# microsoft/tutel

Hardware: AMD Instinct MI355X
Metric: MoE-layer fwd tokens/sec, 4096 tok x H=2048 x E=64 top-2 (higher is better)
Workload: dtype bf16

## Files before the change

### tutel_amd/csrc/common.h

```cpp
#pragma once
#include <hip/hip_runtime.h>
#include <stdint.h>
#include <stdio.h>
#include <string.h>

#include "../../include/tutel_amd.h"

#define WAVE 64

void tutel_set_error(const char *fmt, ...);
int tutel_get_option(int key);

int tutel_stage_begin(int stage, hipStream_t st);
void tutel_stage_end(int token, hipStream_t st);
void tutel_stage_hint(int stage);
void tutel_gemm_corun_hint(int on);
int tutel_gemm_corun();
void tutel_stage_range_push(int stage);
void tutel_stage_range_pop();
struct StageScope {
  int token;
  hipStream_t st;
  StageScope(int stage, hipStream_t s) : token(tutel_stage_begin(stage, s)), st(s) { tutel_stage_range_push(stage); }
  ~StageScope() {
    tutel_stage_end(token, st);
    tutel_stage_range_pop();
  }
};

#define EP_NCAN 16
struct PeerCanary {
  const uint32_t *epoch;
  long long off;
  int world;
  int stale;
};
struct EncodePeer {
  const uint64_t *tab;
  long long off;
  int rank, rows;
  int slot0;
  PeerCanary can;
};
int tutel_encode_launch(const void *x, int dtype, const int32_t *slot_map, const void *gates, int gate_dtype, int T, int M,
                        int n_slots, int capacity, int num_experts, int chunk_rows, int expert_slice, int ep_world, void *out,
                        const EncodePeer &peer, hipStream_t st);
struct GemmProblem {
  const void *A = nullptr; int64_t a_stride_e = 0, a_stride_w = 0; int a_rows_per_w = 0, lda = 0;
  const void *W = nullptr; int64_t w_stride_e = 0; int ldw = 0;
  const void *bias = nullptr; int64_t bias_stride_e = 0;
  void *D = nullptr; int64_t d_stride_e = 0, d_stride_w = 0; int d_rows_per_w = 0, ldd = 0;
  int E_loc = 0, R = 0, N = 0, K = 0;
  int dtype = -1;
  const int32_t *row_counts = nullptr; int row_align = 1;
  const int32_t *a_rows = nullptr; int a_rows_mod = 0; const void *a_zero = nullptr;
  const void *mul = nullptr;
  const uint64_t *d_peer = nullptr; int64_t d_peer_off = 0; const PeerCanary *d_can = nullptr;
  const uint8_t *fl_idx8 = nullptr; int fl_n = 0; int32_t *fl_loc = nullptr;
};
static inline void gemm_one_rank(GemmProblem &g, int R) {
  g.R = R;
  g.a_rows_per_w = g.d_rows_per_w = R > 0 ? R : 1;
}
static inline void gemm_gather(GemmProblem &g, const int32_t *slot_map, int T, const void *zero_row) {
  g.a_rows = slot_map; g.a_rows_mod = slot_map != nullptr ? T : 0; g.a_zero = zero_row;
}
int tutel_expert_gemm(const GemmProblem &g, int w_kmajor, int act, hipStream_t st);
int tutel_expert_ffn(const GemmProblem &fc1, const GemmProblem &fc2, int act, int query, hipStream_t st);
struct RouteFinish;
void tutel_route_finish_args(int T, int E, int k, void *ws, RouteFinish *out);
int tutel_decode_finish_launch(const void *buf, int dtype, const int32_t *idx, const int32_t *loc, const void *gates, int gate_dtype, int T, int M,
                               int k, int capacity, int num_experts, void *out, const RouteFinish &fin, hipStream_t st);
#define PK_TILE_ROWS 256
struct PackedTable { const int32_t *off, *tiles, *ntiles, *cap; int tiles_bound; };
int tutel_expert_gemm_packed(const GemmProblem &g, int w_kmajor, int act, const PackedTable &t, const void *w_up, hipStream_t st);
int tutel_decode_packed_launch(const void *buf, int dtype, const int32_t *idx, const int32_t *loc, const void *gates, int gate_dtype, int T,
                               int M, int k, int row_limit, const int32_t *off, void *out, hipStream_t st);
int tutel_gate_topk_launch(const void *in, const float *partials, int splits, int dtype, int T, int E, int k, int normalize_gate,
                           void *logits_out, int32_t *idx, void *gates, void *ws, int32_t *clear_map, int clear_n, uint8_t *idx8,
                           hipStream_t st);
int tutel_route_launch(const tutel_amd_moe_args_t &m, int splits, int32_t *slot_map, tutel_stream_t stream);
static inline bool gate_proj_mixed(int x_dtype, int logits_dtype) {
  return logits_dtype == TUTEL_F32 && (x_dtype == TUTEL_BF16 || x_dtype == TUTEL_F16);
}
int tutel_gate_proj_splits_for(int T, int M, int E, int x_dtype, int logits_dtype);
int tutel_gate_proj_for(const void *x, const void *gate_w, int x_dtype, int logits_dtype, int T, int M, int E, float *partials,
                        size_t partial_bytes, tutel_stream_t stream);

#define TUTEL_REQUIRE(cond, ...)           \
  do {                                     \
    if (!(cond)) {                         \
      tutel_set_error(__VA_ARGS__);        \
      return -1;                           \
    }                                      \
  } while (0)

#define TUTEL_CHECK_LAUNCH(what)                                                    \
  do {                                                                              \
    hipError_t _e = hipGetLastError();                                              \
    if (_e != hipSuccess) {                                                         \
      tutel_set_error("%s: launch failed: %s", what, hipGetErrorString(_e));        \
      return (int)_e;                                                               \
    }                                                                               \
  } while (0)

struct bf16_t { uint16_t v; };
struct f16_t { _Float16 v; };

__device__ __forceinline__ uint16_t f32_to_bf16_bits(float f) {
  uint32_t u = __float_as_uint(f);
  if ((u & 0x7fffffffu) > 0x7f800000u) return 0x7fc0;
  u += 0x7fffu + ((u >> 16) & 1u);
  return (uint16_t)(u >> 16);
}
__device__ __forceinline__ float bf16_bits_to_f32(uint16_t b) {
  return __uint_as_float(((uint32_t)b) << 16);
}

template <typename T> struct Elem;
template <> struct Elem<double> {
  using ct = double;
  static constexpr int dtype = 3;
  __device__ static __forceinline__ double to_f32(double x) { return x; }
  __device__ static __forceinline__ double from_f32(double x) { return x; }
  __device__ static __forceinline__ double eps() { return 2.220446049250313e-16; }
};
template <> struct Elem<float> {
  using ct = float;
  static constexpr int dtype = TUTEL_F32;
  __device__ static __forceinline__ float to_f32(float x) { return x; }
  __device__ static __forceinline__ float from_f32(float x) { return x; }
  __device__ static __forceinline__ float eps() { return 1.1920928955078125e-07f; }
};
template <> struct Elem<bf16_t> {
  using ct = float;
  static constexpr int dtype = TUTEL_BF16;
  __device__ static __forceinline__ float to_f32(bf16_t x) { return bf16_bits_to_f32(x.v); }
  __device__ static __forceinline__ bf16_t from_f32(float x) { return bf16_t{f32_to_bf16_bits(x)}; }
  __device__ static __forceinline__ float eps() { return 0.0078125f; }
};
template <> struct Elem<f16_t> {
  using ct = float;
  static constexpr int dtype = TUTEL_F16;
  __device__ static __forceinline__ float to_f32(f16_t x) { return (float)x.v; }
  __device__ static __forceinline__ f16_t from_f32(float x) { return f16_t{(_Float16)x}; }
  __device__ static __forceinline__ float eps() { return 0.0009765625f; }
};

template <typename T> __device__ __forceinline__ typename Elem<T>::ct round_to(typename Elem<T>::ct x) {
  return Elem<T>::to_f32(Elem<T>::from_f32(x));
}
__device__ __forceinline__ float ct_exp(float x) { return expf(x); }
__device__ __forceinline__ double ct_exp(double x) { return exp(x); }
__device__ __forceinline__ float ct_max(float a, float b) { return fmaxf(a, b); }
__device__ __forceinline__ double ct_max(double a, double b) { return fmax(a, b); }

static inline int dtype_size(int dtype) { return dtype == TUTEL_F32 ? 4 : 2; }
static inline bool dtype_ok(int dtype) {
  return dtype == TUTEL_F32 || dtype == TUTEL_F16 || dtype == TUTEL_BF16;
}

struct __attribute__((aligned(16))) vec16 { uint32_t w[4]; };

template <typename T> struct Vec;
template <> struct Vec<float> {
  static constexpr int N = 4;
  __device__ static __forceinline__ void unpack(const vec16 &v, float *f) {
#pragma unroll
    for (int i = 0; i < 4; ++i) f[i] = __uint_as_float(v.w[i]);
  }
  __device__ static __forceinline__ void pack(const float *f, vec16 &v) {
#pragma unroll
    for (int i = 0; i < 4; ++i) v.w[i] = __float_as_uint(f[i]);
  }
};
template <> struct Vec<bf16_t> {
  static constexpr int N = 8;
  __device__ static __forceinline__ void unpack(const vec16 &v, float *f) {
#pragma unroll
    for (int i = 0; i < 4; ++i) {
      f[2 * i] = __uint_as_float(v.w[i] << 16);
      f[2 * i + 1] = __uint_as_float(v.w[i] & 0xffff0000u);
    }
  }
  __device__ static __forceinline__ void pack(const float *f, vec16 &v) {
#pragma unroll
    for (int i = 0; i < 4; ++i)
      v.w[i] = (uint32_t)f32_to_bf16_bits(f[2 * i]) | ((uint32_t)f32_to_bf16_bits(f[2 * i + 1]) << 16);
  }
};
template <> struct Vec<f16_t> {
  static constexpr int N = 8;
  __device__ static __forceinline__ void unpack(const vec16 &v, float *f) {
#pragma unroll
    for (int i = 0; i < 4; ++i) {
      union { uint32_t u; _Float16 h[2]; } c;
      c.u = v.w[i];
      f[2 * i] = (float)c.h[0];
      f[2 * i + 1] = (float)c.h[1];
    }
  }
  __device__ static __forceinline__ void pack(const float *f, vec16 &v) {
#pragma unroll
    for (int i = 0; i < 4; ++i) {
      union { uint32_t u; _Float16 h[2]; } c;
      c.h[0] = (_Float16)f[2 * i];
      c.h[1] = (_Float16)f[2 * i + 1];
      v.w[i] = c.u;
    }
  }
};

__device__ __forceinline__ float mul_rn(float a, float b) { return __fmul_rn(a, b); }
__device__ __forceinline__ float add_rn(float a, float b) { return __fadd_rn(a, b); }

__device__ __forceinline__ int lane_id() { return (int)(threadIdx.x & 63); }
__device__ __forceinline__ float wave_max(float v) {
#pragma unroll
  for (int o = 32; o > 0; o >>= 1) v = fmaxf(v, __shfl_xor(v, o, 64));
  return v;
}
__device__ __forceinline__ float wave_sum(float v) {
#pragma unroll
  for (int o = 32; o > 0; o >>= 1) v += __shfl_xor(v, o, 64);
  return v;
}

__device__ __forceinline__ void peer_canary_store(const uint64_t *tab, const PeerCanary &c) {
  if (c.epoch == nullptr) return;
  const int nb = (int)gridDim.x, nlast = nb < EP_NCAN ? nb : EP_NCAN, back = nb - 1 - (int)blockIdx.x;
  if (back >= nlast) return;
  __syncthreads();
  const int t = (int)threadIdx.x;
  if (t >= c.world * EP_NCAN) return;
  const int w = t / EP_NCAN, j = t % EP_NCAN;
  if (j % nlast != back) return;
  const uint32_t e = *c.epoch + (c.stale ? 0u : 1u);
  reinterpret_cast<uint32_t *>(tab[w] + c.off)[j] = e;
}
```

### tutel_amd/csrc/routing.hip

```cpp
#include "common.h"
#include "routing_dev.h"
#include "topk_ties.h"

#define GT_THREADS 1024
#define GT_WAVES 16
#define RT_MAX_TILES 128
#define RT_MAX_K 16
#define RT_MAX_E 4096
#define GT_COL_SLAB 1024

static inline int rt_tile(int T) {
  int per = (T + 64 * RT_MAX_TILES - 1) / (64 * RT_MAX_TILES);
  if (per < 1) per = 1;
  return 64 * per;
}
static inline int rt_ntiles(int T) { return (T + rt_tile(T) - 1) / rt_tile(T); }

extern "C" size_t tutel_amd_routing_workspace_bytes(int T, int E, int k) {
  if (T <= 0 || E <= 0 || k <= 0) return 0;
  size_t nt = (size_t)rt_ntiles(T);
  return nt * ((size_t)k * E * sizeof(int32_t) + (size_t)E * sizeof(float));
}

template <typename T, int EPL, int GT_BATCH>
__global__ __launch_bounds__(GT_THREADS) void gate_topk_kernel(
    const T *__restrict__ in, int apply_softmax, int Tn, int E, int k, int normalize, int tile,
    T *__restrict__ scores_out, int32_t *__restrict__ idx, T *__restrict__ gates,
    int32_t *__restrict__ ws_hist, float *__restrict__ ws_colsum, int32_t *__restrict__ clear_map,
    int clear_n, int tie_mode) {
  using CT = typename Elem<T>::ct;
  extern __shared__ __attribute__((aligned(16))) unsigned char smem[];
  int32_t *s_hist = reinterpret_cast<int32_t *>(smem);
  float *s_col = reinterpret_cast<float *>(smem) + (size_t)k * E;
  const int tie_slots = tie_mode > 0 ? tie_mode : GT_WAVES, tie_slot = (int)(threadIdx.x >> 6) % tie_slots;
  CT *s_tv = reinterpret_cast<CT *>(smem + (((size_t)k * E * 4 + 7) & ~(size_t)7)) + (size_t)tie_slot * E;
  uint16_t *s_tp = reinterpret_cast<uint16_t *>(reinterpret_cast<CT *>(smem + (((size_t)k * E * 4 + 7) & ~(size_t)7)) + (size_t)tie_slots * E) +
                   (size_t)tie_slot * E;
  __shared__ int s_lock[GT_WAVES];

  const int tid = threadIdx.x, lane = tid & 63, wid = tid >> 6;
  const int b = blockIdx.x;
  const int t0 = b * tile, t1 = min(Tn, t0 + tile);

  if (clear_map != nullptr) {
    const int per = (clear_n + (int)gridDim.x - 1) / (int)gridDim.x;
    const int c0 = b * per, c1 = min(clear_n, c0 + per);
    for (int i = c0 + tid; i < c1; i += GT_THREADS) clear_map[i] = -1;
  }

  for (int i = tid; i < k * E; i += GT_THREADS) s_hist[i] = 0;
  if (tid < GT_WAVES) s_lock[tid] = 0;
  __syncthreads();

  float colacc[EPL];
#pragma unroll
  for (int j = 0; j < EPL; ++j) colacc[j] = 0.f;

  for (int tb = t0 + wid; tb < t1; tb += GT_WAVES * GT_BATCH) {
    CT v[GT_BATCH][EPL];
    bool live[GT_BATCH];
    int tt[GT_BATCH];
#pragma unroll
    for (int u = 0; u < GT_BATCH; ++u) {
      tt[u] = tb + u * GT_WAVES;
      live[u] = tt[u] < t1;
      const T *row = in + (size_t)min(tt[u], Tn - 1) * E;
#pragma unroll
      for (int j = 0; j < EPL; ++j) {
        int e = lane + 64 * j;
        v[u][j] = (e < E) ? Elem<T>::to_f32(row[e]) : -INFINITY;
      }
    }
    if (apply_softmax) {
      CT m[GT_BATCH], s[GT_BATCH];
#pragma unroll
      for (int u = 0; u < GT_BATCH; ++u) {
        m[u] = -INFINITY;
#pragma unroll
        for (int j = 0; j < EPL; ++j) m[u] = ct_max(m[u], v[u][j]);
      }
#pragma unroll
      for (int o = 32; o > 0; o >>= 1)
#pragma unroll
        for (int u = 0; u < GT_BATCH; ++u) m[u] = ct_max(m[u], __shfl_xor(m[u], o, 64));
#pragma unroll
      for (int u = 0; u < GT_BATCH; ++u) {
        s[u] = 0.f;
#pragma unroll
        for (int j = 0; j < EPL; ++j) {
          int e = lane + 64 * j;
          v[u][j] = (e < E) ? ct_exp(v[u][j] - m[u]) : 0.f;
          s[u] += v[u][j];
        }
      }
#pragma unroll
      for (int o = 32; o > 0; o >>= 1)
#pragma unroll
        for (int u = 0; u < GT_BATCH; ++u) s[u] += __shfl_xor(s[u], o, 64);
#pragma unroll
      for (int u = 0; u < GT_BATCH; ++u)
#pragma unroll
        for (int j = 0; j < EPL; ++j) {
          int e = lane + 64 * j;
          if (e < E) {
            T r = Elem<T>::from_f32(v[u][j] / s[u]);
            v[u][j] = Elem<T>::to_f32(r);
            if (scores_out && live[u]) scores_out[(size_t)tt[u] * E + e] = r;
          } else {
            v[u][j] = -INFINITY;
          }
        }
    }
    unsigned long long nanm[GT_BATCH];
#pragma unroll
    for (int u = 0; u < GT_BATCH; ++u) {
      nanm[u] = 0;
#pragma unroll
      for (int j = 0; j < EPL; ++j) {
        int e = lane + 64 * j;
        if (e < E && live[u]) colacc[j] += (float)v[u][j];
        if (v[u][j] != v[u][j]) { v[u][j] = -INFINITY; nanm[u] |= 1ull << j; }
      }
    }

    unsigned long long taken[GT_BATCH];
    CT myg[GT_BATCH], prev[GT_BATCH];
    int myidx[GT_BATCH];
    bool tied[GT_BATCH];
#pragma unroll
    for (int u = 0; u < GT_BATCH; ++u) { taken[u] = 0; myg[u] = 0; myidx[u] = -1; prev[u] = 0; tied[u] = false; }
    const int rounds = tie_mode ? k + 1 : k;
    for (int c = 0; c < rounds; ++c) {
      CT bv[GT_BATCH];
      int be[GT_BATCH];
#pragma unroll
      for (int u = 0; u < GT_BATCH; ++u) {
        bv[u] = -INFINITY;
        be[u] = 0x7fffffff;
#pragma unroll
        for (int j = 0; j < EPL; ++j) {
          int e = lane + 64 * j;
          bool ok = (e < E) && !((taken[u] >> j) & 1ull);
          if (ok && (v[u][j] > bv[u] || (v[u][j] == bv[u] && e < be[u]))) { bv[u] = v[u][j]; be[u] = e; }
        }
      }
#pragma unroll
      for (int o = 32; o > 0; o >>= 1)
#pragma unroll
        for (int u = 0; u < GT_BATCH; ++u) {
          CT ov = __shfl_xor(bv[u], o, 64);
          int oe = __shfl_xor(be[u], o, 64);
          if (ov > bv[u] || (ov == bv[u] && oe < be[u])) { bv[u] = ov; be[u] = oe; }
        }
#pragma unroll
      for (int u = 0; u < GT_BATCH; ++u) {
        if (c > 0 && bv[u] == prev[u] && be[u] != 0x7fffffff) tied[u] = true;
        prev[u] = bv[u];
        if (c < k) {
          if ((be[u] & 63) == lane) taken[u] |= 1ull << (be[u] >> 6);
          if (lane == c) { myg[u] = bv[u]; myidx[u] = be[u]; }
        }
      }
    }
    if (tie_mode) {
#pragma unroll
      for (int u = 0; u < GT_BATCH; ++u) {
        if (__ballot(nanm[u] != 0ull) != 0ull) tied[u] = true;
        if (tied[u] && live[u]) {
          const bool shared_slot = tie_slots < GT_WAVES;
          if (shared_slot) {
            if (lane == 0)
              while (atomicCAS(&s_lock[tie_slot], 0, 1) != 0) __builtin_amdgcn_s_sleep(2);
            __builtin_amdgcn_fence(__ATOMIC_ACQUIRE, "workgroup");
            __builtin_amdgcn_wave_barrier();
          }
#pragma unroll
          for (int j = 0; j < EPL; ++j) {
            int e = lane + 64 * j;
            if (e < E) {
              s_tv[e] = ((nanm[u] >> j) & 1ull) ? (CT)NAN : v[u][j];
              s_tp[e] = (uint16_t)e;
            }
          }
          __builtin_amdgcn_fence(__ATOMIC_RELEASE, "wavefront");
          __builtin_amdgcn_wave_barrier();
          if constexpr (EPL <= 4) {
            using Rep = typename TkRepOf<T>::type;
            WaveQueue<EPL, Rep> wq;
            wq.sel = reinterpret_cast<uint8_t *>(s_tp);
            wq.seln = E;
#pragma unroll
            for (int j = 0; j < EPL; ++j) wq.r[j] = Rep::make(((nanm[u] >> j) & 1ull) ? (CT)NAN : v[u][j], lane + 64 * j);
            AtenTopk<WaveQueue<EPL, Rep>> tsw(wq);
            tsw.run(E, k);
            if (lane < k) {
              myidx[u] = Rep::id_of(wq.r[0].unpack());
              myg[u] = s_tv[myidx[u]];
            }
          } else {
            if (lane == 0) {
              LdsQueue<CT, uint16_t> lq{s_tv, s_tp};
              AtenTopk<LdsQueue<CT, uint16_t>> ts(lq);
              ts.run(E, k);
            }
            __builtin_amdgcn_fence(__ATOMIC_ACQ_REL, "wavefront");
            __builtin_amdgcn_wave_barrier();
            if (lane < k) {
              myidx[u] = s_tp[lane];
              myg[u] = s_tv[myidx[u]];
            }
          }
          __builtin_amdgcn_fence(__ATOMIC_ACQ_REL, "wavefront");
          __builtin_amdgcn_wave_barrier();
          if (shared_slot) {
            __builtin_amdgcn_fence(__ATOMIC_RELEASE, "workgroup");
            __builtin_amdgcn_wave_barrier();
            if (lane == 0) __hip_atomic_store(&s_lock[tie_slot], 0, __ATOMIC_RELEASE, __HIP_MEMORY_SCOPE_WORKGROUP);
          }
        }
      }
    }
#pragma unroll
    for (int u = 0; u < GT_BATCH; ++u) {
      CT denom = __shfl(myg[u], 0, 64);
      for (int c = 1; c < k; ++c) denom = round_to<T>(denom + __shfl(myg[u], c, 64));
      if (lane < k && live[u]) {
        CT g = myg[u];
        if (normalize && k > 1) {
          CT d = ct_max(denom, (CT)Elem<T>::eps());
          if (denom != denom) d = denom;
          g = g / d;
        }
        gates[(size_t)lane * Tn + tt[u]] = Elem<T>::from_f32(g);
        idx[(size_t)lane * Tn + tt[u]] = myidx[u];
        atomicAdd(&s_hist[lane * E + myidx[u]], 1);
      }
    }
  }

  __syncthreads();
  for (int i = tid; i < k * E; i += GT_THREADS) ws_hist[(size_t)b * k * E + i] = s_hist[i];
  const int slab = E < GT_COL_SLAB ? E : GT_COL_SLAB;
  for (int e0 = 0; e0 < E; e0 += slab) {
#pragma unroll
    for (int j = 0; j < EPL; ++j) {
      int e = lane + 64 * j;
      if (e >= e0 && e < e0 + slab && e < E) s_col[wid * slab + (e - e0)] = colacc[j];
    }
    __syncthreads();
    for (int e = e0 + tid; e < e0 + slab && e < E; e += GT_THREADS) {
      float s = 0.f;
#pragma unroll
      for (int w = 0; w < GT_WAVES; ++w) s += s_col[w * slab + (e - e0)];
      ws_colsum[(size_t)b * E + e] = s;
    }
    __syncthreads();
  }
}

__global__ __launch_bounds__(RT_THREADS) void tile_hist_kernel(const int32_t *__restrict__ idx,
                                                              int Tn, int E, int k, int tile,
                                                              int32_t *__restrict__ ws_hist) {
  extern __shared__ __attribute__((aligned(16))) unsigned char smem[];
  int32_t *s_hist = reinterpret_cast<int32_t *>(smem);
  const int tid = threadIdx.x, b = blockIdx.x;
  const int t0 = b * tile, t1 = min(Tn, t0 + tile);
  for (int i = tid; i < k * E; i += RT_THREADS) s_hist[i] = 0;
  __syncthreads();
  for (int j = 0; j < k; ++j)
    for (int t = t0 + tid; t < t1; t += RT_THREADS) {
      int e = idx[(size_t)j * Tn + t];
      if (e >= 0 && e < E) atomicAdd(&s_hist[j * E + e], 1);
    }
  __syncthreads();
  for (int i = tid; i < k * E; i += RT_THREADS) ws_hist[(size_t)b * k * E + i] = s_hist[i];
}

template <int NW, bool COH = false>
__device__ __forceinline__ void loc_rank(int tid, int t0, int t1, int Tn, int E, int k, const int32_t *__restrict__ idx,
                                         const int32_t *lidx, int lidx_stride, int e_first, bool have_first, int32_t *s_cur,
                                         int32_t *__restrict__ loc, int capacity, int32_t *__restrict__ slot_map) {
  const int lane = tid & 63, wid = tid >> 6;
  int ebits = 0;
  while ((1 << ebits) < E) ++ebits;
  for (int j = wid; j < k; j += NW) {
    int32_t *cur = s_cur + j * E;
    for (int c0 = t0; c0 < t1; c0 += 64) {
      int t = c0 + lane;
      int e;
      if (have_first && j == wid && c0 == t0) e = e_first;
      else if (t >= t1) e = -1;
      else e = lidx != nullptr ? lidx[j * lidx_stride + (t - t0)] : idx[(size_t)j * Tn + t];
      bool valid = (e >= 0) && (e < E);
      unsigned long long same = __ballot(valid);
      for (int bit = 0; bit < ebits; ++bit) {
        const unsigned long long bb = __ballot(valid && ((e >> bit) & 1));
        same &= ((e >> bit) & 1) ? bb : ~bb;
      }
      const int rank = __popcll(same & ((1ull << lane) - 1ull));
      const int cnt = __popcll(same);
      const bool leader = valid && (__ffsll((long long)same) - 1 == lane);
      int base = valid ? cur[e] : 0;
      int l = base + rank;
      if (leader) cur[e] = base + cnt;
      if (t < t1) {
        loc[(size_t)j * Tn + t] = valid ? l : 0;
        if (slot_map != nullptr && valid && l < capacity) st_i32<COH>(slot_map + (size_t)e * capacity + l, j * Tn + t);
      }
    }
  }
}

__global__ __launch_bounds__(RT_THREADS) void location_kernel(
    const int32_t *__restrict__ idx, int Tn, int E, int k, int tile, int ntiles,
    const int32_t *__restrict__ ws_hist, const float *__restrict__ ws_colsum,
    int32_t *__restrict__ loc, int32_t *__restrict__ dispatch_count, int32_t *__restrict__ stats,
    void *__restrict__ l_aux, int l_aux_dtype, int capacity, int32_t *__restrict__ slot_map) {
  extern __shared__ __attribute__((aligned(16))) unsigned char smem[];
  int32_t *s_cur = reinterpret_cast<int32_t *>(smem);
  int32_t *s_tot = s_cur + (size_t)k * E;
  float *s_parts = reinterpret_cast<float *>(smem) + (size_t)2 * k * E;
  __shared__ float s_red[RT_WAVES];
  __shared__ int s_redi[RT_WAVES];

  const int tid = threadIdx.x, lane = tid & 63, wid = tid >> 6;
  const int b = blockIdx.x;
  const int t0 = b * tile, t1 = min(Tn, t0 + tile);

  int e_first = -1;
  if (wid < k && t0 + lane < t1) e_first = idx[(size_t)wid * Tn + t0 + lane];
  const int cs_parts = (E >= RT_THREADS) ? 1 : (RT_THREADS / E);
  const int cs_per = (ntiles + cs_parts - 1) / cs_parts;
  const bool cs_early = b == 0 && l_aux != nullptr && cs_parts * E <= RT_THREADS;
  float cs_first[16];
  if (cs_early && tid < cs_parts * E) {
    const int e = tid % E, a = (tid / E) * cs_per, z = min(ntiles, a + cs_per);
#pragma unroll
    for (int u = 0; u < 16; ++u) cs_first[u] = (a + u < z) ? ws_colsum[(size_t)(a + u) * E + e] : 0.f;
  }
  loc_prefix<RT_WAVES>(tid, b, E, k, ntiles, ws_hist, s_cur, s_tot, dispatch_count);
  loc_rank<RT_WAVES>(tid, t0, t1, Tn, E, k, idx, nullptr, 0, e_first, true, s_cur, loc, capacity, slot_map);
  if (b == 0) loc_finish<RT_WAVES>(tid, Tn, E, k, ntiles, ws_colsum, s_tot, s_parts, s_red, s_redi, cs_first, cs_early, stats, l_aux, l_aux_dtype);
}

#define GQ_LPT 16
#define GQ_THREADS 1024

template <typename V, int N> struct alignas((sizeof(V) * N) > 16 ? 16 : (sizeof(V) * N)) GqPack { V v[N]; };
template <typename V, int N> __device__ __forceinline__ void gq_load(const V *p, V (&o)[N]) {
  const GqPack<V, N> pk = *reinterpret_cast<const GqPack<V, N> *>(p);
#pragma unroll
  for (int i = 0; i < N; ++i) o[i] = pk.v[i];
}

template <typename T, int EPQ>
__global__ __launch_bounds__(GQ_THREADS) void gate_topk_quad_kernel(
    const T *__restrict__ in, int apply_softmax, int Tn, int E, int k, int normalize, int tile,
    T *__restrict__ scores_out, int32_t *__restrict__ idx, T *__restrict__ gates,
    int32_t *__restrict__ ws_hist, float *__restrict__ ws_colsum, int32_t *__restrict__ clear_map,
    int clear_n, const float *__restrict__ part, int nsplit, T *__restrict__ logits_out, uint8_t *__restrict__ idx8, int tie_mode) {
  using CT = typename Elem<T>::ct;
  extern __shared__ __attribute__((aligned(16))) unsigned char smem[];
  const int ES = GQ_LPT * EPQ + 1;
  int32_t *s_hist = reinterpret_cast<int32_t *>(smem);
  float *s_sc = reinterpret_cast<float *>(smem) + (size_t)k * E;
  CT *s_tv = reinterpret_cast<CT *>(smem + ((((size_t)k * E + (size_t)64 * ES) * 4 + 7) & ~(size_t)7));
  uint8_t *s_sel = reinterpret_cast<uint8_t *>(s_tv + (size_t)64 * E) + (size_t)(threadIdx.x >> 6) * 256;
  __shared__ int s_nlist[2];
  __shared__ int s_list[64];

  const int tid = threadIdx.x, q = tid & (GQ_LPT - 1), tl = tid / GQ_LPT;
  const int b = blockIdx.x;
  const int t0 = b * tile, t1 = min(Tn, t0 + tile);

  if (clear_map != nullptr) {
    const int per = (clear_n + (int)gridDim.x - 1) / (int)gridDim.x;
    const int c0 = b * per, c1 = min(clear_n, c0 + per);
    for (int i = c0 + tid; i < c1; i += GQ_THREADS) clear_map[i] = -1;
  }
  for (int i = tid; i < k * E; i += GQ_THREADS) s_hist[i] = 0;
  if (tid < 2) s_nlist[tid] = 0;
  float colsum = 0.f;
  __syncthreads();

  int pass = -1;
  for (int ts = t0; ts < t1; ts += 64) {
    ++pass;
    const int t = ts + tl;
    const bool live = t < t1;
    CT v[EPQ];
    if (part != nullptr) {
      const float *row = part + (size_t)min(t, Tn - 1) * E + q * EPQ;
      const size_t sstride = (size_t)Tn * E;
      const bool exact = E == GQ_LPT * EPQ;
      int ej[EPQ];
#pragma unroll
      for (int j = 0; j < EPQ; ++j) ej[j] = min(q * EPQ + j, E - 1) - q * EPQ;
      float a[EPQ];
#pragma unroll
      for (int j = 0; j < EPQ; ++j) a[j] = 0.f;
#define GQ_PART_SUM(LOAD)                                                                          \
      for (int s0 = 0; s0 < nsplit; s0 += 4) {                                                     \
        float b[4][EPQ];                                                                           \
        _Pragma("unroll") for (int i = 0; i < 4; ++i) {                                            \
          const float *rs = row + (size_t)min(s0 + i, nsplit - 1) * sstride;                       \
          LOAD;                                                                                    \
        }                                                                                          \
        _Pragma("unroll") for (int i = 0; i < 4; ++i)                                              \
          if (s0 + i < nsplit) {                                                                   \
            _Pragma("unroll") for (int j = 0; j < EPQ; ++j) a[j] = (s0 + i == 0) ? b[i][j] : a[j] + b[i][j]; \
          }                                                                                        \
      }
      if (exact) {
        GQ_PART_SUM((gq_load<float, EPQ>(rs, b[i])));
      } else {
        GQ_PART_SUM(_Pragma("unroll") for (int j = 0; j < EPQ; ++j) b[i][j] = rs[ej[j]]);
      }
#undef GQ_PART_SUM
#pragma unroll
      for (int j = 0; j < EPQ; ++j) {
        int e = q * EPQ + j;
        const T r = Elem<T>::from_f32((CT)a[j]);
        if (logits_out && live && e < E) logits_out[(size_t)t * E + e] = r;
        v[j] = (e < E) ? Elem<T>::to_f32(r) : -INFINITY;
      }
    } else {
      const T *row = in + (size_t)min(t, Tn - 1) * E + q * EPQ;
      T raw[EPQ];
      if (E == GQ_LPT * EPQ && (reinterpret_cast<uintptr_t>(in) & 15) == 0) {
        gq_load<T, EPQ>(row, raw);
      } else {
#pragma unroll
        for (int j = 0; j < EPQ; ++j) raw[j] = row[min(q * EPQ + j, E - 1) - q * EPQ];
      }
#pragma unroll
      for (int j = 0; j < EPQ; ++j) {
        int e = q * EPQ + j;
        v[j] = (e < E) ? Elem<T>::to_f32(raw[j]) : -INFINITY;
      }
    }
    if (apply_softmax) {
      CT m = -INFINITY;
#pragma unroll
      for (int j = 0; j < EPQ; ++j) m = ct_max(m, v[j]);
#pragma unroll
      for (int o = 1; o < GQ_LPT; o <<= 1) m = ct_max(m, __shfl_xor(m, o, 64));
      CT s = 0;
#pragma unroll
      for (int j = 0; j < EPQ; ++j) {
        int e = q * EPQ + j;
        v[j] = (e < E) ? ct_exp(v[j] - m) : CT(0);
        s += v[j];
      }
#pragma unroll
      for (int o = 1; o < GQ_LPT; o <<= 1) s += __shfl_xor(s, o, 64);
#pragma unroll
      for (int j = 0; j < EPQ; ++j) {
        int e = q * EPQ + j;
        if (e < E) {
          T r = Elem<T>::from_f32(v[j] / s);
          v[j] = Elem<T>::to_f32(r);
          if (scores_out && live) scores_out[(size_t)t * E + e] = r;
        } else {
          v[j] = -INFINITY;
        }
      }
    }
    uint32_t nanm = 0;
#pragma unroll
    for (int j = 0; j < EPQ; ++j) {
      int e = q * EPQ + j;
      if (e < E) s_sc[tl * ES + e] = live ? (float)v[j] : 0.f;
      if (v[j] != v[j]) { v[j] = -INFINITY; nanm |= 1u << j; }
    }

    uint32_t taken = 0;
    CT myg = 0, prev = 0;
    int myidx = 0;
    bool tied = false;
    const int rounds = tie_mode ? k + 1 : k;
    for (int c = 0; c < rounds; ++c) {
      CT bv = -INFINITY;
      int be = 0x7fffffff;
#pragma unroll
      for (int j = 0; j < EPQ; ++j) {
        int e = q * EPQ + j;
        bool ok = (e < E) && !((taken >> j) & 1u);
        if (ok && (v[j] > bv || (v[j] == bv && e < be))) { bv = v[j]; be = e; }
      }
#pragma unroll
      for (int o = 1; o < GQ_LPT; o <<= 1) {
        CT ov = __shfl_xor(bv, o, 64);
        int oe = __shfl_xor(be, o, 64);
        if (ov > bv || (ov == bv && oe < be)) { bv = ov; be = oe; }
      }
      if (c > 0 && bv == prev && be != 0x7fffffff) tied = true;
      prev = bv;
      if (c < k) {
        if (be / EPQ == q) taken |= 1u << (be - q * EPQ);
        if (c == q) { myg = bv; myidx = be; }
        if (q == 0 && live) {
          idx[(size_t)c * Tn + t] = be;
          if (idx8 != nullptr) idx8[(size_t)c * Tn + t] = (uint8_t)be;
        }
      }
    }
    if (tie_mode) {
      const int rowsh = (int)(threadIdx.x & 48);
      if ((__ballot(nanm != 0) >> rowsh) & 0xffffull) tied = true;
      if (tied && live) {
#pragma unroll
        for (int j = 0; j < EPQ; ++j) {
          int e = q * EPQ + j;
          if (e < E) s_tv[tl * E + e] = ((nanm >> j) & 1u) ? (CT)NAN : v[j];
        }
        if (q == 0) s_list[atomicAdd(&s_nlist[pass & 1], 1)] = tl;
      }
    }
    {
      const int row0 = (int)(threadIdx.x & 48);
      CT denom = __shfl(myg, row0, 64);
      for (int c = 1; c < k; ++c) denom = round_to<T>(denom + __shfl(myg, row0 + c, 64));
      if (q < k && live && !(tie_mode && tied)) {
        CT g = myg;
        if (normalize && k > 1) {
          CT d = ct_max(denom, (CT)Elem<T>::eps());
          if (denom != denom) d = denom;
          g = g / d;
        }
        gates[(size_t)q * Tn + t] = Elem<T>::from_f32(g);
        atomicAdd(&s_hist[q * E + myidx], 1);
      }
    }
    __syncthreads();
    if (tid < E) {
      float s = colsum;
      for (int r = 0; r < 64; ++r) s += s_sc[r * ES + tid];
      colsum = s;
    }
    if (tie_mode) {
      const int wv = (int)(threadIdx.x >> 6), nbusy = (E + 63) >> 6, wl = (int)(threadIdx.x & 63);
      constexpr int SL = (GQ_LPT * EPQ + 63) / 64;
      const int nrep = s_nlist[pass & 1];
      for (int ent = wv - nbusy; ent >= 0 && ent < nrep; ent += GQ_THREADS / 64 - nbusy) {
        const int trow = s_list[ent], tt = ts + trow;
        using Rep = typename TkRepOf<T>::type;
        WaveQueue<SL, Rep> wq;
        wq.sel = s_sel;
        wq.seln = E;
#pragma unroll
        for (int sl = 0; sl < SL; ++sl) {
          const int e = wl + 64 * sl;
          wq.r[sl] = Rep::make(e < E ? s_tv[trow * E + e] : (CT)0, e);
        }
        AtenTopk<WaveQueue<SL, Rep>> tk(wq);
        tk.run(E, k);
        TkElem<CT> res;
        res.id = Rep::id_of(wq.r[0].unpack());
        res.v = s_tv[trow * E + (wl < k ? res.id : 0)];
        CT denom = tk_readlane(res.v, 0);
        for (int c = 1; c < k; ++c) denom = round_to<T>(denom + tk_readlane(res.v, c));
        if (wl < k) {
          CT g = res.v;
          if (normalize && k > 1) {
            CT d = ct_max(denom, (CT)Elem<T>::eps());
            if (denom != denom) d = denom;
            g = g / d;
          }
          gates[(size_t)wl * Tn + tt] = Elem<T>::from_f32(g);
          idx[(size_t)wl * Tn + tt] = res.id;
          if (idx8 != nullptr) idx8[(size_t)wl * Tn + tt] = (uint8_t)res.id;
          atomicAdd(&s_hist[wl * E + res.id], 1);
        }
      }
      if (tid == 0) s_nlist[(pass + 1) & 1] = 0;
    }
    __syncthreads();
  }
  for (int i = tid; i < k * E; i += GQ_THREADS) ws_hist[(size_t)b * k * E + i] = s_hist[i];
  if (tid < E) ws_colsum[(size_t)b * E + tid] = colsum;
}

__global__ __launch_bounds__(256) void slot_map_kernel(const int32_t *__restrict__ idx,
                                                       const int32_t *__restrict__ loc, int n,
                                                       int E, int capacity,
                                                       int32_t *__restrict__ slot_map) {
  int q = blockIdx.x * 256 + threadIdx.x;
  if (q >= n) return;
  int e = idx[q], l = loc[q];
  if (e >= 0 && e < E && l >= 0 && l < capacity) slot_map[(size_t)e * capacity + l] = q;
}

#define CS_WAVES 16
__global__ __launch_bounds__(CS_WAVES * 64) void cumsum_kernel(const int32_t *__restrict__ in,
                                                              int32_t *__restrict__ out, int Tn,
                                                              int E) {
  __shared__ int32_t s_part[CS_WAVES][64];
  const int lane = threadIdx.x & 63, wid = threadIdx.x >> 6;
  const int col = blockIdx.x * 64 + lane;
  const int rows_per = (Tn + CS_WAVES - 1) / CS_WAVES;
  const int r0 = wid * rows_per, r1 = min(Tn, r0 + rows_per);
  int acc = 0;
  if (col < E)
    for (int r = r0; r < r1; ++r) acc += in[(size_t)r * E + col];
  s_part[wid][lane] = acc;
  __syncthreads();
  int run = -1;
  for (int w = 0; w < wid; ++w) run += s_part[w][lane];
  if (col < E)
    for (int r = r0; r < r1; ++r) {
      run += in[(size_t)r * E + col];
      out[(size_t)r * E + col] = run;
    }
}

template <typename T>
static int launch_gate_topk(const void *in, int apply_softmax, int Tn, int E, int k, int normalize,
                            void *scores_out, int32_t *idx, void *gates, void *ws,
                            int32_t *clear_map, int clear_n, hipStream_t st, const float *part = nullptr, int nsplit = 0,
                            void *logits_out = nullptr, uint8_t *idx8 = nullptr) {
  const int tile = rt_tile(Tn), nt = rt_ntiles(Tn);
  int32_t *ws_hist = (int32_t *)ws;
  float *ws_col = (float *)(ws_hist + (size_t)nt * k * E);
  using CTh = typename Elem<T>::ct;
  int tie_mode = tutel_get_option(TUTEL_OPT_TIE_RULE) != 0;
  size_t lds = (size_t)k * E * 4 + 8;
  {
    const size_t col = (size_t)GT_WAVES * (E < GT_COL_SLAB ? E : GT_COL_SLAB) * 4, slot = (size_t)E * (sizeof(CTh) + 2);
    const size_t room = (size_t)160 * 1024 - lds - 256;
    int slots = (int)(room / slot);
    if (slots > GT_WAVES) slots = GT_WAVES;
    if (slots < 1) tie_mode = 0;
    const size_t tie = tie_mode ? (size_t)slots * slot : 0;
    lds += tie > col ? tie : col;
    if (tie_mode && E > 128) tie_mode = slots;
  }
  if (E <= 128) {
    const int epq = (E + GQ_LPT - 1) / GQ_LPT;
    const int epq_t = epq <= 1 ? 1 : (epq <= 2 ? 2 : (epq <= 4 ? 4 : 8));
    const size_t lds_q = ((size_t)k * E + (size_t)64 * (GQ_LPT * epq_t + 1)) * 4 + 8 + (tie_mode ? (size_t)64 * E * sizeof(CTh) + 16 * 256 : 0);
#define GQ_LAUNCH(EPQ)                                                                         \
    do {                                                                                       \
      if (lds_q > 65536) {                                                                     \
        (void)hipFuncSetAttribute((const void *)gate_topk_quad_kernel<T, EPQ>, hipFuncAttributeMaxDynamicSharedMemorySize, (int)lds_q); \
        (void)hipGetLastError();                                                               \
      }                                                                                        \
      hipLaunchKernelGGL((gate_topk_quad_kernel<T, EPQ>), dim3(nt), dim3(GQ_THREADS), lds_q, st,            \
                         (const T *)in, apply_softmax, Tn, E, k, normalize, tile, (T *)scores_out,          \
                         idx, (T *)gates, ws_hist, ws_col, clear_map, clear_n, part, nsplit, (T *)logits_out, idx8, tie_mode); \
    } while (0)
    if (epq_t == 1) GQ_LAUNCH(1);
    else if (epq_t == 2) GQ_LAUNCH(2);
    else if (epq_t == 4) GQ_LAUNCH(4);
    else GQ_LAUNCH(8);
#undef GQ_LAUNCH
    TUTEL_CHECK_LAUNCH("tutel_amd_gate_topk");
    return 0;
  }
  TUTEL_REQUIRE(part == nullptr && idx8 == nullptr, "tutel_amd_gate_topk_partials: E = %d is past the 128 experts the partial-sum form covers", E);
  const int epl = (E + 63) / 64;
#define GT_LAUNCH(EPL)                                                                          \
  do {                                                                                          \
    if (lds > 65536) {                                                                          \
      (void)hipFuncSetAttribute((const void *)gate_topk_kernel<T, EPL, (EPL <= 4 ? 4 : (EPL <= 8 ? 2 : 1))>,                         \
                                hipFuncAttributeMaxDynamicSharedMemorySize, (int)lds);          \
      (void)hipGetLastError();                                                                  \
    }                                                                                           \
    hipLaunchKernelGGL((gate_topk_kernel<T, EPL, (EPL <= 4 ? 4 : (EPL <= 8 ? 2 : 1))>), dim3(nt), dim3(GT_THREADS), lds, st,         \
                       (const T *)in, apply_softmax, Tn, E, k, normalize, tile,                 \
                       (T *)scores_out, idx, (T *)gates, ws_hist, ws_col, clear_map, clear_n, tie_mode);  \
  } while (0)
  if (epl <= 1) GT_LAUNCH(1);
  else if (epl <= 2) GT_LAUNCH(2);
  else if (epl <= 4) GT_LAUNCH(4);
  else if (epl <= 8) GT_LAUNCH(8);
  else if (epl <= 16) GT_LAUNCH(16);
  else if (epl <= 32) GT_LAUNCH(32);
  else GT_LAUNCH(64);
#undef GT_LAUNCH
  TUTEL_CHECK_LAUNCH("tutel_amd_gate_topk");
  return 0;
}

extern "C" int tutel_amd_gate_topk(const void *in, int dtype, int apply_softmax, int T, int E,
                                   int k, int normalize_gate, void *scores_out, int32_t *idx,
                                   void *gates, void *ws, size_t ws_bytes, int32_t *clear_map,
                                   int clear_n, tutel_stream_t stream) {
  TUTEL_REQUIRE(dtype_ok(dtype) || dtype == TUTEL_F64, "tutel_amd_gate_topk: unsupported dtype %d", dtype);
  TUTEL_REQUIRE(T >= 0 && E >= 1 && E <= RT_MAX_E, "tutel_amd_gate_topk: need 1 <= E <= %d (got %d)", RT_MAX_E, E);
  TUTEL_REQUIRE(k >= 1 && k <= RT_MAX_K && k <= E, "tutel_amd_gate_topk: need 1 <= k <= min(E,%d) (got k=%d, E=%d)", RT_MAX_K, k, E);
  TUTEL_REQUIRE((size_t)k * E <= 8192, "tutel_amd_gate_topk: k*E = %d exceeds 8192", k * E);
  if (T == 0) return 0;
  TUTEL_REQUIRE(in && idx && gates && ws, "tutel_amd_gate_topk: null pointer");
  TUTEL_REQUIRE(ws_bytes >= tutel_amd_routing_workspace_bytes(T, E, k), "tutel_amd_gate_topk: workspace too small");
  TUTEL_REQUIRE(clear_n >= 0 && (clear_map != nullptr || clear_n == 0), "tutel_amd_gate_topk: bad clear_map");
  if (clear_n == 0) clear_map = nullptr;
  hipStream_t st = (hipStream_t)stream;
  StageScope stage(TUTEL_STAGE_GATE_TOPK, st);
  if (dtype == TUTEL_F64) return launch_gate_topk<double>(in, apply_softmax, T, E, k, normalize_gate, scores_out, idx, gates, ws, clear_map, clear_n, st);
  if (dtype == TUTEL_F32) return launch_gate_topk<float>(in, apply_softmax, T, E, k, normalize_gate, scores_out, idx, gates, ws, clear_map, clear_n, st);
  if (dtype == TUTEL_BF16) return launch_gate_topk<bf16_t>(in, apply_softmax, T, E, k, normalize_gate, scores_out, idx, gates, ws, clear_map, clear_n, st);
  return launch_gate_topk<f16_t>(in, apply_softmax, T, E, k, normalize_gate, scores_out, idx, gates, ws, clear_map, clear_n, st);
}

void tutel_route_finish_args(int T, int E, int k, void *ws, RouteFinish *out) {
  const int nt = rt_ntiles(T);
  out->Tn = T; out->E = E; out->k = k; out->ntiles = nt;
  out->ws_hist = (const int32_t *)ws;
  out->ws_colsum = (const float *)((const int32_t *)ws + (size_t)nt * k * E);
}

int tutel_gate_topk_launch(const void *in, const float *partials, int splits, int dtype, int T, int E, int k, int normalize_gate,
                           void *logits_out, int32_t *idx, void *gates, void *ws, int32_t *clear_map, int clear_n, uint8_t *idx8,
                           hipStream_t st) {
  TUTEL_REQUIRE(E <= 128 || (partials == nullptr && idx8 == nullptr), "tutel_gate_topk_launch: E = %d is past the 16-lanes-per-token kernel", E);
  if (clear_n == 0) clear_map = nullptr;
  StageScope stage(TUTEL_STAGE_GATE_TOPK, st);
  const int sm = 1;
  if (dtype == TUTEL_F32) return launch_gate_topk<float>(in, sm, T, E, k, normalize_gate, nullptr, idx, gates, ws, clear_map, clear_n, st, partials, splits, logits_out, idx8);
  if (dtype == TUTEL_BF16) return launch_gate_topk<bf16_t>(in, sm, T, E, k, normalize_gate, nullptr, idx, gates, ws, clear_map, clear_n, st, partials, splits, logits_out, idx8);
  return launch_gate_topk<f16_t>(in, sm, T, E, k, normalize_gate, nullptr, idx, gates, ws, clear_map, clear_n, st, partials, splits, logits_out, idx8);
}

extern "C" int tutel_amd_gate_topk_partials(const float *partials, int splits, int dtype, int T, int E, int k,
                                            int normalize_gate, void *logits_out, void *scores_out, int32_t *idx,
                                            void *gates, void *ws, size_t ws_bytes, int32_t *clear_map, int clear_n,
                                            tutel_stream_t stream) {
  TUTEL_REQUIRE(dtype_ok(dtype), "tutel_amd_gate_topk_partials: the logits dtype must be fp32 / fp16 / bf16 (got %d)", dtype);
  TUTEL_REQUIRE(T >= 0 && E >= 1 && E <= 128, "tutel_amd_gate_topk_partials: need 1 <= E <= 128 (got %d)", E);
  TUTEL_REQUIRE(k >= 1 && k <= RT_MAX_K && k <= E, "tutel_amd_gate_topk_partials: need 1 <= k <= min(E,%d) (got k=%d, E=%d)", RT_MAX_K, k, E);
  TUTEL_REQUIRE(splits >= 1 && splits <= 64, "tutel_amd_gate_topk_partials: bad split count %d", splits);
  if (T == 0) return 0;
  TUTEL_REQUIRE(partials && idx && gates && ws, "tutel_amd_gate_topk_partials: null pointer");
  TUTEL_REQUIRE(ws_bytes >= tutel_amd_routing_workspace_bytes(T, E, k), "tutel_amd_gate_topk_partials: workspace too small");
  TUTEL_REQUIRE(clear_n >= 0 && (clear_map != nullptr || clear_n == 0), "tutel_amd_gate_topk_partials: bad clear_map");
  if (clear_n == 0) clear_map = nullptr;
  hipStream_t st = (hipStream_t)stream;
  StageScope stage(TUTEL_STAGE_GATE_TOPK, st);
  if (dtype == TUTEL_F32)
    return launch_gate_topk<float>(nullptr, 1, T, E, k, normalize_gate, scores_out, idx, gates, ws, clear_map, clear_n, st, partials, splits, logits_out);
  if (dtype == TUTEL_BF16)
    return launch_gate_topk<bf16_t>(nullptr, 1, T, E, k, normalize_gate, scores_out, idx, gates, ws, clear_map, clear_n, st, partials, splits, logits_out);
  return launch_gate_topk<f16_t>(nullptr, 1, T, E, k, normalize_gate, scores_out, idx, gates, ws, clear_map, clear_n, st, partials, splits, logits_out);
}

extern "C" int tutel_amd_compute_location(const int32_t *idx, int T, int E, int k, int hist_ready,
                                          void *ws, size_t ws_bytes, int32_t *loc,
                                          int32_t *dispatch_count, int32_t *stats, void *l_aux,
                                          int l_aux_dtype, int capacity, int32_t *slot_map,
                                          int slot_map_cleared, tutel_stream_t stream) {
  TUTEL_REQUIRE(T >= 0 && E >= 1 && E <= RT_MAX_E, "tutel_amd_compute_location: need 1 <= E <= %d (got %d)", RT_MAX_E, E);
  TUTEL_REQUIRE(k >= 1 && k <= RT_MAX_K, "tutel_amd_compute_location: need 1 <= k <= %d (got %d)", RT_MAX_K, k);
  TUTEL_REQUIRE((size_t)k * E <= 8192, "tutel_amd_compute_location: k*E = %d exceeds 8192", k * E);
  TUTEL_REQUIRE(dispatch_count != nullptr, "tutel_amd_compute_location: dispatch_count is null");
  TUTEL_REQUIRE(l_aux == nullptr || dtype_ok(l_aux_dtype), "tutel_amd_compute_location: bad l_aux dtype %d", l_aux_dtype);
  TUTEL_REQUIRE((long long)k * T < 0x7fffffffLL, "tutel_amd_compute_location: k*T overflows int32");
  TUTEL_REQUIRE(hist_ready || l_aux == nullptr, "tutel_amd_compute_location: l_aux needs the column sums written by tutel_amd_gate_topk (hist_ready=1)");
  hipStream_t st = (hipStream_t)stream;
  if (T == 0) {
    (void)hipMemsetAsync(dispatch_count, 0, (size_t)E * 4, st);
    if (stats) (void)hipMemsetAsync(stats, 0, 4, st);
    if (l_aux) (void)hipMemsetAsync(l_aux, 0, dtype_size(l_aux_dtype), st);
    if (slot_map && capacity > 0) (void)hipMemsetAsync(slot_map, 0xFF, (size_t)E * capacity * 4, st);
    return 0;
  }
  TUTEL_REQUIRE(idx && loc && ws, "tutel_amd_compute_location: null pointer");
  TUTEL_REQUIRE(ws_bytes >= tutel_amd_routing_workspace_bytes(T, E, k), "tutel_amd_compute_location: workspace too small");
  const int tile = rt_tile(T), nt = rt_ntiles(T);
  int32_t *ws_hist = (int32_t *)ws;
  float *ws_col = (float *)(ws_hist + (size_t)nt * k * E);
  StageScope stage(TUTEL_STAGE_LOCATION, st);
  if (!hist_ready) {
    hipLaunchKernelGGL(tile_hist_kernel, dim3(nt), dim3(RT_THREADS), (size_t)k * E * 4, st, idx, T, E, k, tile, ws_hist);
    TUTEL_CHECK_LAUNCH("tutel_amd_compute_location(hist)");
  }
  if (slot_map != nullptr && capacity > 0) {
    if (!slot_map_cleared) {
      hipError_t e = hipMemsetAsync(slot_map, 0xFF, (size_t)E * capacity * 4, st);
      TUTEL_REQUIRE(e == hipSuccess, "tutel_amd_compute_location: memset failed: %s", hipGetErrorString(e));
    }
  } else {
    slot_map = nullptr;
    capacity = 0;
  }
  const size_t lds_loc = ((size_t)2 * k * E + (size_t)(E > RT_THREADS ? E : RT_THREADS)) * 4;
  if (lds_loc > 65536) {
    (void)hipFuncSetAttribute((const void *)location_kernel, hipFuncAttributeMaxDynamicSharedMemorySize, (int)lds_loc);
    (void)hipGetLastError();
  }
  hipLaunchKernelGGL(location_kernel, dim3(nt), dim3(RT_THREADS), lds_loc, st, idx, T, E, k,
                     tile, nt, ws_hist, ws_col, loc, dispatch_count, stats, l_aux, l_aux_dtype, capacity, slot_map);
  TUTEL_CHECK_LAUNCH("tutel_amd_compute_location");
  return 0;
}

extern "C" int tutel_amd_slot_map(const int32_t *idx, const int32_t *loc, int T, int E, int k,
                                  int capacity, int32_t *slot_map, tutel_stream_t stream) {
  TUTEL_REQUIRE(E >= 1 && k >= 1 && capacity >= 0 && T >= 0, "tutel_amd_slot_map: bad sizes");
  TUTEL_REQUIRE((long long)k * T < 0x7fffffffLL, "tutel_amd_slot_map: k*T overflows int32");
  hipStream_t st = (hipStream_t)stream;
  if (capacity == 0) return 0;
  TUTEL_REQUIRE(slot_map != nullptr, "tutel_amd_slot_map: null slot_map");
  StageScope stage(TUTEL_STAGE_OTHER, st);
  hipError_t e = hipMemsetAsync(slot_map, 0xFF, (size_t)E * capacity * 4, st);
  TUTEL_REQUIRE(e == hipSuccess, "tutel_amd_slot_map: memset failed: %s", hipGetErrorString(e));
  int n = k * T;
  if (n == 0) return 0;
  TUTEL_REQUIRE(idx && loc, "tutel_amd_slot_map: null pointer");
  hipLaunchKernelGGL(slot_map_kernel, dim3((n + 255) / 256), dim3(256), 0, st, idx, loc, n, E, capacity, slot_map);
  TUTEL_CHECK_LAUNCH("tutel_amd_slot_map");
  return 0;
}

extern "C" int tutel_amd_cumsum_sub_one(const int32_t *mask, int32_t *out, int T, int E,
                                        tutel_stream_t stream) {
  TUTEL_REQUIRE(T >= 0 && E >= 0, "tutel_amd_cumsum_sub_one: bad sizes");
  if (T == 0 || E == 0) return 0;
  TUTEL_REQUIRE(mask && out, "tutel_amd_cumsum_sub_one: null pointer");
  hipLaunchKernelGGL(cumsum_kernel, dim3((E + 63) / 64), dim3(CS_WAVES * 64), 0, (hipStream_t)stream, mask, out, T, E);
  TUTEL_CHECK_LAUNCH("tutel_amd_cumsum_sub_one");
  return 0;
}
```

Before: 16.79 million.

## Prefetch gate rows across passes, use DPP row reductions in top-k kernel

Hoists the per-pass row loads for gate logits and partial sums so that the first pass's loads are issued before the shared-memory clear and each later pass issues its loads at the top of the loop. The 16-lane shuffle reductions for softmax max/sum and the top-k argmax are replaced with DPP row moves (quad xor and row mirrors). The extra tie-detection round is replaced by a ballot check on the remaining candidates. The normalization denominator is now accumulated inside the selection loop rather than gathered by shuffles afterwards. The aim is lower latency in a small routing kernel, at the cost of more live registers and the added complexity of macros and DPP intrinsics.

```diff
diff --git a/tutel_amd/csrc/common.h b/tutel_amd/csrc/common.h
--- a/tutel_amd/csrc/common.h
+++ b/tutel_amd/csrc/common.h
@@ -226,6 +226,23 @@
   return v;
 }
 
+#define DPP_QUAD_XOR1 0xB1
+#define DPP_QUAD_XOR2 0x4E
+#define DPP_ROW_HALF_MIRROR 0x141
+#define DPP_ROW_MIRROR 0x140
+template <int CTRL> __device__ __forceinline__ int dpp_row_move(int x) { return __builtin_amdgcn_update_dpp(0, x, CTRL, 0xf, 0xf, true); }
+template <int CTRL> __device__ __forceinline__ float dpp_row_move(float x) { return __int_as_float(dpp_row_move<CTRL>(__float_as_int(x))); }
+template <int CTRL> __device__ __forceinline__ double dpp_row_move(double x) {
+  return __hiloint2double(dpp_row_move<CTRL>(__double2hiint(x)), dpp_row_move<CTRL>(__double2loint(x)));
+}
+template <typename V, typename Op> __device__ __forceinline__ V row16_all_reduce(V x, Op op) {
+  x = op(x, dpp_row_move<DPP_QUAD_XOR1>(x));
+  x = op(x, dpp_row_move<DPP_QUAD_XOR2>(x));
+  x = op(x, dpp_row_move<DPP_ROW_HALF_MIRROR>(x));
+  x = op(x, dpp_row_move<DPP_ROW_MIRROR>(x));
+  return x;
+}
+
 __device__ __forceinline__ void peer_canary_store(const uint64_t *tab, const PeerCanary &c) {
   if (c.epoch == nullptr) return;
   const int nb = (int)gridDim.x, nlast = nb < EP_NCAN ? nb : EP_NCAN, back = nb - 1 - (int)blockIdx.x;
diff --git a/tutel_amd/csrc/routing.hip b/tutel_amd/csrc/routing.hip
--- a/tutel_amd/csrc/routing.hip
+++ b/tutel_amd/csrc/routing.hip
@@ -353,6 +353,15 @@
   for (int i = 0; i < N; ++i) o[i] = pk.v[i];
 }
 
+template <typename CT> struct GqBest { CT v; int e; };
+template <typename CT> __device__ __forceinline__ GqBest<CT> gq_better(GqBest<CT> a, GqBest<CT> o) {
+  const bool take = (o.v > a.v) | ((o.v == a.v) & (o.e < a.e));
+  return GqBest<CT>{take ? o.v : a.v, take ? o.e : a.e};
+}
+template <int CTRL, typename CT> __device__ __forceinline__ GqBest<CT> dpp_row_move(GqBest<CT> x) {
+  return GqBest<CT>{dpp_row_move<CTRL>(x.v), dpp_row_move<CTRL>(x.e)};
+}
+
 template <typename T, int EPQ>
 __global__ __launch_bounds__(GQ_THREADS) void gate_topk_quad_kernel(
     const T *__restrict__ in, int apply_softmax, int Tn, int E, int k, int normalize, int tile,
@@ -373,6 +382,35 @@
   const int b = blockIdx.x;
   const int t0 = b * tile, t1 = min(Tn, t0 + tile);
 
+  const size_t sstride = (size_t)Tn * E;
+  const bool exact = E == GQ_LPT * EPQ;
+  const bool wide_in = exact && (reinterpret_cast<uintptr_t>(in) & 15) == 0;
+  int ej[EPQ];
+#pragma unroll
+  for (int j = 0; j < EPQ; ++j) ej[j] = min(q * EPQ + j, E - 1) - q * EPQ;
+  float pb[4][EPQ];
+  T raw[EPQ];
+#define GQ_PART_LOAD(S0, LOAD)                                                                     \
+  _Pragma("unroll") for (int i = 0; i < 4; ++i) {                                                  \
+    const float *rs = row + (size_t)min((S0) + i, nsplit - 1) * sstride;                           \
+    LOAD;                                                                                          \
+  }
+#define GQ_LOAD_WIDE gq_load<float, EPQ>(rs, pb[i])
+#define GQ_LOAD_ELEMS _Pragma("unroll") for (int j = 0; j < EPQ; ++j) pb[i][j] = rs[ej[j]]
+#define GQ_PASS_LOADS(TS)                                                                          \
+  do {                                                                                             \
+    const size_t roff = (size_t)min((TS) + tl, Tn - 1) * E + q * EPQ;                              \
+    if (part != nullptr) {                                                                         \
+      const float *row = part + roff;                                                              \
+      if (exact) { GQ_PART_LOAD(0, GQ_LOAD_WIDE) } else { GQ_PART_LOAD(0, GQ_LOAD_ELEMS) }         \
+    } else if (wide_in) {                                                                          \
+      gq_load<T, EPQ>(in + roff, raw);                                                             \
+    } else {                                                                                       \
+      _Pragma("unroll") for (int j = 0; j < EPQ; ++j) raw[j] = in[roff + ej[j]];                   \
+    }                                                                                              \
+  } while (0)
+  GQ_PASS_LOADS(t0);
+
   if (clear_map != nullptr) {
     const int per = (clear_n + (int)gridDim.x - 1) / (int)gridDim.x;
     const int c0 = b * per, c1 = min(clear_n, c0 + per);
@@ -385,38 +423,27 @@
 
   int pass = -1;
   for (int ts = t0; ts < t1; ts += 64) {
-    ++pass;
+    if (++pass > 0) GQ_PASS_LOADS(ts);
     const int t = ts + tl;
     const bool live = t < t1;
     CT v[EPQ];
     if (part != nullptr) {
       const float *row = part + (size_t)min(t, Tn - 1) * E + q * EPQ;
-      const size_t sstride = (size_t)Tn * E;
-      const bool exact = E == GQ_LPT * EPQ;
-      int ej[EPQ];
-#pragma unroll
-      for (int j = 0; j < EPQ; ++j) ej[j] = min(q * EPQ + j, E - 1) - q * EPQ;
       float a[EPQ];
 #pragma unroll
       for (int j = 0; j < EPQ; ++j) a[j] = 0.f;
-#define GQ_PART_SUM(LOAD)                                                                          \
-      for (int s0 = 0; s0 < nsplit; s0 += 4) {                                                     \
-        float b[4][EPQ];                                                                           \
-        _Pragma("unroll") for (int i = 0; i < 4; ++i) {                                            \
-          const float *rs = row + (size_t)min(s0 + i, nsplit - 1) * sstride;                       \
-          LOAD;                                                                                    \
-        }                                                                                          \
-        _Pragma("unroll") for (int i = 0; i < 4; ++i)                                              \
-          if (s0 + i < nsplit) {                                                                   \
-            _Pragma("unroll") for (int j = 0; j < EPQ; ++j) a[j] = (s0 + i == 0) ? b[i][j] : a[j] + b[i][j]; \
-          }                                                                                        \
-      }
+#define GQ_PART_ADD(S0)                                                                           \
+      _Pragma("unroll") for (int i = 0; i < 4; ++i)                                                \
+        if ((S0) + i < nsplit) {                                                                   \
+          _Pragma("unroll") for (int j = 0; j < EPQ; ++j) a[j] = ((S0) + i == 0) ? pb[i][j] : a[j] + pb[i][j]; \
+        }
+      GQ_PART_ADD(0)
       if (exact) {
-        GQ_PART_SUM((gq_load<float, EPQ>(rs, b[i])));
+        for (int s0 = 4; s0 < nsplit; s0 += 4) { GQ_PART_LOAD(s0, GQ_LOAD_WIDE) GQ_PART_ADD(s0) }
       } else {
-        GQ_PART_SUM(_Pragma("unroll") for (int j = 0; j < EPQ; ++j) b[i][j] = rs[ej[j]]);
-      }
-#undef GQ_PART_SUM
+        for (int s0 = 4; s0 < nsplit; s0 += 4) { GQ_PART_LOAD(s0, GQ_LOAD_ELEMS) GQ_PART_ADD(s0) }
+      }
+#undef GQ_PART_ADD
 #pragma unroll
       for (int j = 0; j < EPQ; ++j) {
         int e = q * EPQ + j;
@@ -425,14 +452,6 @@
         v[j] = (e < E) ? Elem<T>::to_f32(r) : -INFINITY;
       }
     } else {
-      const T *row = in + (size_t)min(t, Tn - 1) * E + q * EPQ;
-      T raw[EPQ];
-      if (E == GQ_LPT * EPQ && (reinterpret_cast<uintptr_t>(in) & 15) == 0) {
-        gq_load<T, EPQ>(row, raw);
-      } else {
-#pragma unroll
-        for (int j = 0; j < EPQ; ++j) raw[j] = row[min(q * EPQ + j, E - 1) - q * EPQ];
-      }
 #pragma unroll
       for (int j = 0; j < EPQ; ++j) {
         int e = q * EPQ + j;
@@ -443,8 +462,7 @@
       CT m = -INFINITY;
 #pragma unroll
       for (int j = 0; j < EPQ; ++j) m = ct_max(m, v[j]);
-#pragma unroll
-      for (int o = 1; o < GQ_LPT; o <<= 1) m = ct_max(m, __shfl_xor(m, o, 64));
+      m = row16_all_reduce(m, [](CT x, CT y) { return ct_max(x, y); });
       CT s = 0;
 #pragma unroll
       for (int j = 0; j < EPQ; ++j) {
@@ -452,8 +470,7 @@
         v[j] = (e < E) ? ct_exp(v[j] - m) : CT(0);
         s += v[j];
       }
-#pragma unroll
-      for (int o = 1; o < GQ_LPT; o <<= 1) s += __shfl_xor(s, o, 64);
+      s = row16_all_reduce(s, [](CT x, CT y) { return x + y; });
 #pragma unroll
       for (int j = 0; j < EPQ; ++j) {
         int e = q * EPQ + j;
@@ -475,39 +492,36 @@
     }
 
     uint32_t taken = 0;
-    CT myg = 0, prev = 0;
+    CT myg = 0, prev = 0, denom = 0;
     int myidx = 0;
     bool tied = false;
-    const int rounds = tie_mode ? k + 1 : k;
-    for (int c = 0; c < rounds; ++c) {
-      CT bv = -INFINITY;
-      int be = 0x7fffffff;
+    for (int c = 0; c < k; ++c) {
+      GqBest<CT> best{-INFINITY, 0x7fffffff};
 #pragma unroll
       for (int j = 0; j < EPQ; ++j) {
         int e = q * EPQ + j;
         bool ok = (e < E) && !((taken >> j) & 1u);
-        if (ok && (v[j] > bv || (v[j] == bv && e < be))) { bv = v[j]; be = e; }
-      }
-#pragma unroll
-      for (int o = 1; o < GQ_LPT; o <<= 1) {
-        CT ov = __shfl_xor(bv, o, 64);
-        int oe = __shfl_xor(be, o, 64);
-        if (ov > bv || (ov == bv && oe < be)) { bv = ov; be = oe; }
-      }
-      if (c > 0 && bv == prev && be != 0x7fffffff) tied = true;
+        best = gq_better(best, GqBest<CT>{ok ? v[j] : (CT)-INFINITY, ok ? e : 0x7fffffff});
+      }
+      best = row16_all_reduce(best, [](GqBest<CT> x, GqBest<CT> y) { return gq_better(x, y); });
+      const CT bv = best.v;
+      const int be = best.e;
+      if (c > 0 && bv == prev) tied = true;
       prev = bv;
-      if (c < k) {
-        if (be / EPQ == q) taken |= 1u << (be - q * EPQ);
-        if (c == q) { myg = bv; myidx = be; }
-        if (q == 0 && live) {
-          idx[(size_t)c * Tn + t] = be;
-          if (idx8 != nullptr) idx8[(size_t)c * Tn + t] = (uint8_t)be;
-        }
+      denom = c == 0 ? bv : round_to<T>(denom + bv);
+      if (be / EPQ == q) taken |= 1u << (be - q * EPQ);
+      if (c == q) { myg = bv; myidx = be; }
+      if (q == 0 && live) {
+        idx[(size_t)c * Tn + t] = be;
+        if (idx8 != nullptr) idx8[(size_t)c * Tn + t] = (uint8_t)be;
       }
     }
     if (tie_mode) {
+      bool more = nanm != 0;
+#pragma unroll
+      for (int j = 0; j < EPQ; ++j) more |= (q * EPQ + j < E) & !((taken >> j) & 1u) & (v[j] == prev);
       const int rowsh = (int)(threadIdx.x & 48);
-      if ((__ballot(nanm != 0) >> rowsh) & 0xffffull) tied = true;
+      if ((__ballot(more) >> rowsh) & 0xffffull) tied = true;
       if (tied && live) {
 #pragma unroll
         for (int j = 0; j < EPQ; ++j) {
@@ -518,9 +532,6 @@
       }
     }
     {
-      const int row0 = (int)(threadIdx.x & 48);
-      CT denom = __shfl(myg, row0, 64);
-      for (int c = 1; c < k; ++c) denom = round_to<T>(denom + __shfl(myg, row0 + c, 64));
       if (q < k && live && !(tie_mode && tied)) {
         CT g = myg;
         if (normalize && k > 1) {
@@ -579,6 +590,10 @@
   }
   for (int i = tid; i < k * E; i += GQ_THREADS) ws_hist[(size_t)b * k * E + i] = s_hist[i];
   if (tid < E) ws_colsum[(size_t)b * E + tid] = colsum;
+#undef GQ_PASS_LOADS
+#undef GQ_LOAD_ELEMS
+#undef GQ_LOAD_WIDE
+#undef GQ_PART_LOAD
 }
 
 __global__ __launch_bounds__(256) void slot_map_kernel(const int32_t *__restrict__ idx,
```

After: 16.85 million (median of 6 runs). Within noise of the previous version (+0.3%).
